# Eddie-Wang1120/Eddie-Wang-Hackathon2023

Measured on AMD Instinct MI355X. Metric: decode tokens/s, whole job (encoder + cross-KV + language-ID + prefill + greedy decode), Whisper large-v2 int8 weight-only + int8 KV; rtf reported beside it, higher is better.
Workload: dtype f16

## Files before the change

### eddie-wang-hackathon2023_amd/csrc/decoder.hip

```cpp
#include <stdio.h>
#include <string.h>

#include <atomic>

#include "engine_internal.h"

using namespace wm;

namespace {
constexpr int MAX_DEVICES = 64;
struct Profiler {
    bool enabled = false; int layer_stride = 1;
    std::vector<hipEvent_t> start, stop; size_t used = 0;
    long long* timeline = nullptr; int timeline_cap = 0;
};
std::mutex g_prof_mu;
Profiler g_prof_dev[MAX_DEVICES];
int current_device_index() {
    int dev = 0;
    if (hipGetDevice(&dev) != hipSuccess || dev < 0 || dev >= MAX_DEVICES) dev = 0;
    return dev;
}

int prof_slot(Profiler& pr, int layer, hipStream_t s) {
// ... 671 lines not shown

int wm_stream_destroy(wm_stream_t stream) {
    if (stream) WM_CHECK_HIP(hipStreamDestroy((hipStream_t)stream));
    return 0;
}

int wm_profile_configure(int enabled, int layer_stride, int max_samples) {
    WM_REQUIRE(layer_stride >= 1 && max_samples >= 0, "wm_profile_configure: bad arguments");
    std::lock_guard<std::mutex> lock(g_prof_mu);
    Profiler& g_prof = g_prof_dev[current_device_index()];
    g_prof.enabled = false;
    for (size_t i = 0; i < g_prof.start.size(); ++i) { (void)hipEventDestroy(g_prof.start[i]); (void)hipEventDestroy(g_prof.stop[i]); }
    g_prof.start.clear(); g_prof.stop.clear(); g_prof.used = 0; g_prof.layer_stride = layer_stride;
    if (!enabled) return 0;
    g_prof.start.resize(max_samples); g_prof.stop.resize(max_samples);
    for (int i = 0; i < max_samples; ++i) {
        WM_CHECK_HIP(hipEventCreate(&g_prof.start[i]));
        WM_CHECK_HIP(hipEventCreate(&g_prof.stop[i]));
    }
    g_prof.enabled = true;
    return 0;
}

int wm_debug_timeline(void* buf, int capacity) {
    std::lock_guard<std::mutex> lock(g_prof_mu);
    Profiler& pr = g_prof_dev[current_device_index()];
    pr.timeline = (long long*)buf;
    pr.timeline_cap = buf ? capacity : 0;
    return 0;
}

int wm_profile_read(double* total_ms, int64_t* count, int reset) {
    WM_REQUIRE(total_ms && count, "wm_profile_read: null argument");
    std::lock_guard<std::mutex> lock(g_prof_mu);
    Profiler& g_prof = g_prof_dev[current_device_index()];
    double sum = 0.0;
    for (size_t i = 0; i < g_prof.used; ++i) {
        float ms = 0.f;
        WM_CHECK_HIP(hipEventSynchronize(g_prof.stop[i]));
        WM_CHECK_HIP(hipEventElapsedTime(&ms, g_prof.start[i], g_prof.stop[i]));
        sum += ms;
    }
    *total_ms = sum; *count = (int64_t)g_prof.used;
    if (reset) g_prof.used = 0;
    return 0;
}

int wm_greedy_step(const wm_greedy_io* io, wm_stream_t stream) {
    WM_REQUIRE(io && io->logits && io->tokens && io->sum_logprobs, "wm_greedy_step: null argument");
    GreedyParams p{};
    p.logits = (h16*)io->logits; p.ld_row = io->row_stride; p.B = io->batch; p.V = io->n_vocab;
    p.tokens = io->tokens; p.ld_tok = io->tokens_ld; p.cur_len = io->cur_len; p.sum_logprobs = io->sum_logprobs;
    p.suppress = io->suppress; p.n_suppress = io->n_suppress; p.blank = io->blank; p.n_blank = io->n_blank;
    p.sample_begin = io->sample_begin; p.eot = io->eot; p.timestamp_begin = io->timestamp_begin;
    p.max_initial_ts = io->max_initial_timestamp_index; p.apply_rules = io->apply_rules; p.n_done = io->n_done;
    p.t_dev = io->n_past_dev;
    p.done = io->done; p.row_limit = io->row_limit;
    WM_REQUIRE(io->temperature >= 0.f, "wm_greedy_step: negative temperature");
    p.temperature = io->temperature; p.seed_lo = (uint32_t)io->seed; p.seed_hi = (uint32_t)(io->seed >> 32);
    p.seed_dev = io->seed_dev; p.row0 = io->row0;
    return launch_greedy(p, (hipStream_t)stream);
}

int wm_step_advance(int32_t* counter, wm_stream_t stream) { return launch_step_advance(counter, (hipStream_t)stream); }
int wm_step_finish(int32_t* counter, const int32_t* done, int batch, int32_t* live, wm_stream_t stream) {
    return launch_step_finish(counter, done, batch, live, (hipStream_t)stream);
}
int wm_step_finish_group(int32_t* counter, const int32_t* done, int batch, int group, int32_t* live, int32_t* live_groups, wm_stream_t stream) {
    return launch_step_finish_group(counter, done, batch, group, live, live_groups, (hipStream_t)stream);
}

int wm_set_rows_path(int min_rows) {
    const int prev = rows_path_min_rows();
    g_rows_min.store(min_rows < 0 ? 0 : min_rows, std::memory_order_relaxed);
    return prev;
}

int wm_set_gemm_small_tiles(int tiles) {
    const int prev = get_gemm_small_tiles();
    set_gemm_small_tiles(tiles);
    return prev;
}

int wm_set_self_attn_waves(int waves) {
    self_attn_waves(1);
    const int prev = g_self_waves.load(std::memory_order_relaxed);
    g_self_waves.store(waves == 1 || waves == 4 ? waves : 0, std::memory_order_relaxed);
    return prev;
}

int wm_set_small_batch_rows(int rows) {
    const int prev = small_path_max_rows();
    g_small_rows.store(rows < 0 ? 0 : (rows > GEMV_SMALL_MAX_M ? GEMV_SMALL_MAX_M : rows), std::memory_order_relaxed);
    return prev;
}

int wm_set_decode_chain(int on) {
    const int prev = g_decode_chain.load(std::memory_order_relaxed);
    g_decode_chain.store(on < 0 ? DECODE_CHAIN_DEFAULT : (on > 2 ? 2 : on), std::memory_order_relaxed);
    for (ChainDev& cd : g_chain_dev) {
        std::lock_guard<std::mutex> lk(cd.mu);
        if (cd.declined) { cd.declined = false; cd.reason.clear(); }
    }
    return prev;
}

int wm_decode_chain_error(int* out) {
    WM_REQUIRE(out, "wm_decode_chain_error: null argument");
    ChainDev& cd = chain_dev_slot(current_device_index());
    const unsigned v = chain_err_peek(cd);
    *out = (int)v;
    if (v) {
        std::lock_guard<std::mutex> lk(cd.mu);
        __atomic_store_n(cd.err_host, 0u, __ATOMIC_RELAXED);
        cd.declined = true;
        cd.reason = "a one-launch decode step gave up waiting for its workgroups (they were not resident together)";
    }
    return 0;
}

int wm_decode_chain_status(wm_chain_status* out) {
    WM_REQUIRE(out, "wm_decode_chain_status: null argument");
    ChainDev& cd = chain_dev_slot(current_device_index());
    std::lock_guard<std::mutex> lk(cd.mu);
    memset(out, 0, sizeof(*out));
    out->mode = g_decode_chain.load(std::memory_order_relaxed);
    out->launches = cd.launches.load(std::memory_order_relaxed);
    out->declined_calls = cd.declined_calls.load(std::memory_order_relaxed);
    out->declined = cd.declined ? 1 : 0;
    out->error_pending = chain_err_peek(cd) ? 1 : 0;
    snprintf(out->reason, sizeof(out->reason), "%s", cd.reason.c_str());
    snprintf(out->footprint, sizeof(out->footprint), "%s", cd.footprint.c_str());
    return 0;
}

int wm_set_cross_v_skip(int on) {
    const int prev = g_cross_v_skip.load(std::memory_order_relaxed);
    g_cross_v_skip.store(on < 0 ? CROSS_V_SKIP_DEFAULT : (on ? 1 : 0), std::memory_order_relaxed);
    return prev;
}

}
```

### eddie-wang-hackathon2023_amd/csrc/gemm_f16.hip

```cpp
#include <stdlib.h>

#include <atomic>

#include "common.h"
#include "kernels.h"

namespace wm {

namespace f16gemm {
constexpr int BK = 64;
}

template <int NWAVE, int BN, int ACT>
__global__ __launch_bounds__(NWAVE * 64, 2) void gemm_f16_kernel(GemmBigParams p) {
    using namespace f16gemm;
    constexpr int TM = 4, ROWS_W = 16 * TM;
    constexpr int BM = NWAVE / 2 * ROWS_W;
    static_assert((BM + BN) / 8 % NWAVE == 0, "DMA pieces must divide evenly over the waves");
    constexpr int A_STAGE = BM * BK * 2, B_STAGE = BN * BK * 2, STAGE = A_STAGE + B_STAGE;
    constexpr int LOADS = (BM + BN) / 8 / NWAVE;
    constexpr int TN = BN / 2 / 16;
    extern __shared__ __attribute__((aligned(1024))) unsigned char smem[];

    const int tid = threadIdx.x, lane = tid & 63, wid = tid >> 6;
// ... 73 lines not shown

    constexpr int WN_COLS = BN / 2;
    const bool scale_cols = p.colscale_n > 0;
    half4v b4[TN];
#pragma unroll
    for (int j = 0; j < TN; ++j) {
        const int col = col0 + wc * WN_COLS + j * 16 + g * 4;
        b4[j] = p.bias ? *(const half4v*)(p.bias + col) : half4v{0, 0, 0, 0};
    }
    const int colw = col0 + wc * WN_COLS + g * 4;
#pragma unroll
    for (int i = 0; i < TM; ++i) {
        const int row = row0 + wr * ROWS_W + i * 16 + (lane & 15);
        const int rowc = row < p.M ? row : p.M - 1;
        half4v r4[TN];
        if (p.residual) {
            const h16* rrow = p.residual + (size_t)(p.res_mod > 0 ? rowc % p.res_mod : rowc) * p.ldr + colw;
#pragma unroll
            for (int j = 0; j < TN; ++j) r4[j] = *(const half4v*)(rrow + j * 16);
        }
        float v[TN][4];
#pragma unroll
        for (int j = 0; j < TN; ++j)
#pragma unroll
            for (int r = 0; r < 4; ++r) v[j][r] = r16_f32(acc[i][j][r] + (float)b4[j][r]);
        if (ACT == 1) {
#pragma unroll
            for (int j = 0; j < TN; ++j)
#pragma unroll
                for (int r = 0; r < 4; ++r) v[j][r] = r16_f32(gelu_erf(v[j][r]));
        } else if (ACT == 2) {
#pragma unroll
            for (int j = 0; j < TN; ++j)
#pragma unroll
                for (int r = 0; r < 4; ++r) v[j][r] = r16_f32(gelu_tanh(v[j][r]));
        }
        if (scale_cols) {
#pragma unroll
            for (int j = 0; j < TN; ++j) {
                const float sc = (colw + j * 16 < p.colscale_n) ? p.colscale : 1.0f;
#pragma unroll
                for (int r = 0; r < 4; ++r) v[j][r] = r16_f32(v[j][r] * sc);
            }
        }
        if (p.residual) {
#pragma unroll
            for (int j = 0; j < TN; ++j)
#pragma unroll
                for (int r = 0; r < 4; ++r) v[j][r] += (float)r4[j][r];
        }
        if (row >= p.M) continue;
        if (p.out_mode == 0) {
            h16* crow = p.C + (p.c_rows > 0 ? (size_t)(row / p.c_rows) * p.c_bstride + (size_t)(row % p.c_rows) * p.ldc
                                            : (size_t)row * p.ldc) + colw;
#pragma unroll
            for (int j = 0; j < TN; ++j)
                *(half4v*)(crow + j * 16) = half4v{(h16)v[j][0], (h16)v[j][1], (h16)v[j][2], (h16)v[j][3]};
        } else {
            const int HC = p.hs_H * 64;
            const int bb = row / p.hs_T, t = row % p.hs_T;
#pragma unroll
            for (int j = 0; j < TN; ++j) {
                const int col = colw + j * 16;
                const int kv = p.hs_kv < 0 ? col / HC : p.hs_kv, cc = p.hs_kv < 0 ? col % HC : col;
                const size_t off = ((((size_t)bb * 2 + kv) * p.hs_H + (cc >> 6)) * p.hs_T + t) * 64 + (cc & 63);
                if (p.q8_inv_scale > 0.f) {
                    char4 q;
                    q.x = (signed char)fminf(127.f, fmaxf(-128.f, rintf(r16(v[j][0]) * p.q8_inv_scale)));
                    q.y = (signed char)fminf(127.f, fmaxf(-128.f, rintf(r16(v[j][1]) * p.q8_inv_scale)));
                    q.z = (signed char)fminf(127.f, fmaxf(-128.f, rintf(r16(v[j][2]) * p.q8_inv_scale)));
                    q.w = (signed char)fminf(127.f, fmaxf(-128.f, rintf(r16(v[j][3]) * p.q8_inv_scale)));
                    *(char4*)((signed char*)p.C + off) = q;
                } else
                *(half4v*)(p.C + off) = half4v{(h16)v[j][0], (h16)v[j][1], (h16)v[j][2], (h16)v[j][3]};
            }
        }
    }
}

static std::atomic<int> g_small_tiles{GEMM_SMALL_TILES_DEFAULT};
void set_gemm_small_tiles(int tiles) { g_small_tiles.store(tiles > 0 ? tiles : (tiles == 0 ? 0 : GEMM_SMALL_TILES_DEFAULT), std::memory_order_relaxed); }
int get_gemm_small_tiles() { return g_small_tiles.load(std::memory_order_relaxed); }

int launch_gemm_f16(const GemmBigParams& p, hipStream_t stream) {
    using namespace f16gemm;
    const bool few = p.max_wgs <= 0 && p.N % 128 == 0 &&
                     (long)((p.M + 255) / 256) * ((p.N + 255) / 256) < (long)g_small_tiles.load(std::memory_order_relaxed);
    if (!few && gemm_f16p_supports(p)) return launch_gemm_f16p(p, stream);
    WM_REQUIRE(p.N % 128 == 0, "gemm_f16: N=%d must be a multiple of 128", p.N);
    WM_REQUIRE(p.K % BK == 0, "gemm_f16: K=%d must be a multiple of %d", p.K, BK);
    WM_REQUIRE(p.lda % 8 == 0, "gemm_f16: lda=%d must be a multiple of 8 (16-byte loads)", p.lda);
    WM_REQUIRE(p.ldc % 4 == 0 && p.ldr % 4 == 0, "gemm_f16: ldc/ldr must be multiples of 4 (8-byte epilogue accesses)");
    WM_REQUIRE(p.M > 0, "gemm_f16: empty M");
    WM_REQUIRE(p.act >= 0 && p.act <= 2, "gemm_f16: act=%d", p.act);
    static const int tiny_max = lab_env_int("WM_GEMM_TINY_TILES", GEMM_TINY_TILES_DEFAULT);
    const long tiles128 = (long)((p.M + 127) / 128) * (p.N / 128);
    const int form = few ? (tiles128 <= tiny_max ? 3 : 2) : (p.N % 256 == 0 ? 0 : 1);
    const int bm = form == 3 ? 64 : (form == 2 ? 128 : 256), bn = form == 0 ? 256 : 128;
    const int grid = ((p.M + bm - 1) / bm) * (p.N / bn);
    static std::atomic<unsigned long long> attr_set{0};
    int dev = 0;
    WM_CHECK_HIP(hipGetDevice(&dev));
    const int slot = dev & 63;
    using Kern = void (*)(GemmBigParams);
    static const Kern kerns[4][3] = {{gemm_f16_kernel<8, 256, 0>, gemm_f16_kernel<8, 256, 1>, gemm_f16_kernel<8, 256, 2>},
                                     {gemm_f16_kernel<8, 128, 0>, gemm_f16_kernel<8, 128, 1>, gemm_f16_kernel<8, 128, 2>},
                                     {gemm_f16_kernel<4, 128, 0>, gemm_f16_kernel<4, 128, 1>, gemm_f16_kernel<4, 128, 2>},
                                     {gemm_f16_kernel<2, 128, 0>, gemm_f16_kernel<2, 128, 1>, gemm_f16_kernel<2, 128, 2>}};
    static const int rows_of[4] = {256, 256, 128, 64}, cols_of[4] = {256, 128, 128, 128};
    const unsigned long long bit = 1ull << slot;
    if (!(attr_set.load(std::memory_order_acquire) & bit)) {
        for (int f = 0; f < 4; ++f)
            for (int a = 0; a < 3; ++a)
                WM_CHECK_HIP(hipFuncSetAttribute((const void*)kerns[f][a], hipFuncAttributeMaxDynamicSharedMemorySize,
                                                 2 * (rows_of[f] + cols_of[f]) * BK * 2));
        attr_set.fetch_or(bit, std::memory_order_release);
    }
    const size_t lds = (size_t)2 * (bm + bn) * BK * 2;
    hipLaunchKernelGGL(kerns[form][p.act], dim3(grid), dim3(form == 3 ? 128 : (form == 2 ? 256 : 512)), lds, stream, p);
    WM_LAUNCH_CHECK(stream, "gemm_f16");
    return 0;
}

__global__ void dequant_w8_kernel(const int8_t* q, const h16* scale, h16* out, int N, int K) {
    const size_t total = (size_t)N * K / 8;
    for (size_t i = blockIdx.x * (size_t)blockDim.x + threadIdx.x; i < total; i += (size_t)gridDim.x * blockDim.x) {
        const size_t e = i * 8;
        const h16 s = scale[e / K];
        const uint2 w = *(const uint2*)(q + e);
        half2v h[4];
        cvt_s8x4_f16x4(w.x, h[0], h[1]);
        cvt_s8x4_f16x4(w.y, h[2], h[3]);
        half8v o;
#pragma unroll
        for (int j = 0; j < 4; ++j) { o[2 * j] = h[j][0] * s; o[2 * j + 1] = h[j][1] * s; }
        *(half8v*)(out + e) = o;
    }
}

int launch_dequant_w8(const int8_t* q, const h16* scale, h16* out, int N, int K, hipStream_t stream) {
    WM_REQUIRE(K % 8 == 0, "dequant_w8: K=%d must be a multiple of 8", K);
    hipLaunchKernelGGL(dequant_w8_kernel, dim3(2048), dim3(256), 0, stream, q, scale, out, N, K);
    WM_LAUNCH_CHECK(stream, "dequant_w8");
    return 0;
}

}
```

### eddie-wang-hackathon2023_amd/csrc/kernels.h

```cpp
#pragma once
#include "common.h"

namespace wm {

struct GemmBigParams {
    const h16* A; int lda; int M; int K;
    const void* W; int N;
    const h16* bias;
    h16* C; int ldc;
    const h16* residual; int ldr; int res_mod;
    int act;
    int colscale_n; float colscale;
    int out_mode;
    int hs_T, hs_H, hs_kv;
    float q8_inv_scale;
    int a_rows; long a_bstride;
    int c_rows; long c_bstride;
    int max_wgs;
    int nt_flags;
    int tile_rows;
};
int launch_gemm_f16(const GemmBigParams& p, hipStream_t stream);
constexpr int GEMM_SMALL_TILES_DEFAULT = 150;
constexpr int GEMM_TINY_TILES_DEFAULT = 160;
void set_gemm_small_tiles(int tiles);
int get_gemm_small_tiles();
int launch_gemm_f16p(const GemmBigParams& p, hipStream_t stream);
bool gemm_f16p_supports(const GemmBigParams& p);
int launch_dequant_w8(const int8_t* q, const h16* scale, h16* out, int N, int K, hipStream_t stream);

struct GemmSkinnyParams {
    const h16* A; int lda; int M; int K;
    const void* Wt; int n_blocks; int w8;
    const h16* scale;
    int ksplit;
    float* part;
    long part_sstride;
    h16* out; int ldc; int n_valid;
};
constexpr int SKINNY_MAX_M = 256;
int launch_gemm_skinny(const GemmSkinnyParams& p, hipStream_t stream);
int skinny_default_ksplit(int M, int K, int n_blocks, int w8);

struct GemvSmallParams {
    const h16* A; int lda; int M; int K;
    const void* Wt; int n_blocks; int w8;
    const h16* scale;
    int ksplit;
    const h16* ln_g; const h16* ln_b;
    int mode;
    const h16* bias; int gelu_kind;
    float* out32; int ld32;
    h16* out16; int ld16; int n_valid;
    h16* x; int ldx;
};
constexpr int GEMV_SMALL_MAX_M = 32;
int launch_gemv_small(const GemvSmallParams& p, hipStream_t stream);

constexpr int CHAIN_MAX_STAGES = 6;
constexpr int CHAIN_MAX_ROWS = 8;
constexpr int DECODE_CHAIN_DEFAULT = 2;
struct ChainStage {
    const void* Wt; const h16* scale; const h16* bias;
    const h16* ln_g; const h16* ln_b;
    int K, n_blocks;
    int mode;
    int pad_;
};
struct ChainLayerStatic { const h16* qkv_bias; const h16* cq_bias; float kv_scale; int pad_; };
struct ChainLayerIo { const void* cross_kv; void* cache; };
struct GemvChainParams {
    int n_stages; const ChainStage* st;
    float* out32;
    int w8, gelu_kind;
    h16* x;
    unsigned long long* gran_x; unsigned long long* gran_h;
    const h16* cross_kv; int cross_Tk, cross_heads, cross_nsplit; const h16* cross_qbias;
    unsigned long long* gran_q;
    int cross_at, merge_at, merge_nsplit, merge_heads;
    unsigned long long* gran_p;
    const float* self_part; const h16* self_bias; void* self_cache; int self_cap, self_T, self_heads, self_i8; const int32_t* self_t_dev;
    float self_kv_scale; h16* self_out; unsigned long long* gran_c;
    int n_layers; const ChainLayerStatic* lstat; const ChainLayerIo* lio; unsigned long long* gran_s;
    int rows; long cross_row_bytes, self_row_bytes;
    const int32_t* live;
    unsigned* err;
    const unsigned* generation; int launch_id;
};
bool gemv_chain_supports(int C, int w8, int n_cu);
int gemv_chain_resident(int w8, int self_i8, int rows, int cross_Tk, int cross_nsplit, int n_wg, int n_cu, bool* ok, char* why, size_t why_cap);
int launch_occupy(int n_wg, size_t lds_bytes, long long usec, hipStream_t stream);
int launch_gemv_chain(const GemvChainParams& p, const ChainStage* host_stages, int n_wg, hipStream_t stream);
int launch_chain_io_table(ChainLayerIo* dst, const ChainLayerIo* host, int n, hipStream_t stream);

bool gemm_rows_supports(int K, int w8);
int launch_gemm_rows(const GemvSmallParams& p, hipStream_t stream);

struct RowFinishParams {
    const float* part; int ksplit; int M; int N; int ldp;
    long part_sstride;
    const h16* bias;
    int mode; int gelu_kind;
    h16* x; int ldx;
    const h16* ln_g; const h16* ln_b;
    h16* out; int ldo;
    int eager;
};
int launch_row_finish(const RowFinishParams& p, hipStream_t stream);

struct EmbedParams {
    const int32_t* tokens; int tokens_ld;
// ... 127 lines not shown
```

### eddie-wang-hackathon2023_amd/native.py

```python
from __future__ import annotations

import atexit
import ctypes as C
import os
from typing import Optional, Sequence

import sys
import warnings


def _hip_already_initialised() -> bool:
    t = sys.modules.get("torch")
    try:
        return bool(t is not None and t.cuda.is_initialized())
    except Exception:
        return False


def _configure_runtime() -> dict:
    name = "DEBUG_CLR_GRAPH_PACKET_CAPTURE"
    late = _hip_already_initialised()
    if name in os.environ:
        return {"name": name, "value": os.environ[name], "set_by": "caller", "in_time": None}
    if os.environ.get("WM_GRAPH_NODE_REPLAY", "1") == "0":
        return {"name": name, "value": None, "set_by": "nobody (WM_GRAPH_NODE_REPLAY=0)", "in_time": None}
    os.environ[name] = "0"
    if late:
        warnings.warn("whisper_mi355: the HIP runtime was initialised before this package was imported, so "
                      f"{name}=0 (node-by-node graph replay, 6-10 % of the small-batch token step) is NOT in effect: "
                      "import the package before the first torch.cuda call, or export the variable yourself", RuntimeWarning, stacklevel=3)
    return {"name": name, "value": "0", "set_by": "package", "in_time": not late}


RUNTIME_KNOBS = _configure_runtime()


def runtime_report() -> dict:
    rep = dict(RUNTIME_KNOBS)
    rep["effective_env"] = os.environ.get(RUNTIME_KNOBS["name"])
    if _lib is not None:
        buf = C.create_string_buffer(4096)
        _lib.wm_lab_knobs(buf, 4096)
        rep["lab_knobs_honoured"] = buf.value.decode() or None
    return rep


_HERE = os.path.dirname(os.path.abspath(__file__))
LIB_PATH = os.environ.get("WM_LIBRARY_PATH") or os.path.join(_HERE, "libwhisper_mi355.so")

EXPORTS = (
    "wm_version", "wm_last_error", "wm_device_count", "wm_engine_create", "wm_engine_destroy",
    "wm_engine_info", "wm_engine_weight_bytes", "wm_encoder_workspace_bytes", "wm_encoder_forward",
    "wm_encoder_forward_shared", "wm_encoder_forward_range",
    "wm_cross_kv_workspace_bytes", "wm_cross_kv", "wm_decoder_workspace_bytes", "wm_decoder_step",
    "wm_greedy_step", "wm_gemm", "wm_gemm_skinny", "wm_gemm_skinny_default_ksplit", "wm_layernorm",
    "wm_attn_encoder", "wm_attn_decode_cross", "wm_attn_decode_self", "wm_quantize_i8",
    "wm_profile_configure", "wm_profile_read", "wm_step_advance", "wm_log_mel_workspace_bytes", "wm_log_mel",
    "wm_flac_info", "wm_flac_decode", "wm_conv1d_gelu", "wm_argmax", "wm_gemv_fused", "wm_gemm_rows", "wm_set_rows_path", "wm_set_small_batch_rows", "wm_set_self_attn_waves", "wm_set_gemm_small_tiles", "wm_lab_knobs", "wm_set_cross_v_skip", "wm_set_decode_chain", "wm_decode_chain_error", "wm_decode_chain_status", "wm_debug_occupy", "wm_decoder_step_multi", "wm_stream_create_cu_mask", "wm_stream_destroy", "wm_attn_decode_cross_i8", "wm_debug_timeline",
    "wm_step_finish",
    "wm_beam_workspace_bytes", "wm_beam_step", "wm_kv_reorder",
    "wm_gemm_ex", "wm_row_finish", "wm_embed", "wm_mel_transpose_pad", "wm_zero_pad_rows",
    "wm_decoder_step_tap", "wm_align_workspace_bytes", "wm_align", "wm_dtw_workspace_bytes", "wm_dtw",
    "wm_mel_windows", "wm_resample", "wm_attn_decode_self_rows",
    "wm_attn_self_ex", "wm_attn_cross_ex",
    "wm_forced_probs",
    "wm_section_cuts_workspace_bytes", "wm_section_cuts",
    "wm_step_finish_group", "wm_attn_cross_group_ex", "wm_decoder_step_group",
    "wm_decoder_prefill_workspace_bytes", "wm_decoder_prefill", "wm_attn_prefill_self", "wm_attn_prefill_cross",
)


ABI_VERSION = 8

import threading as _threading
CAPTURE_LOCK = _threading.RLock()


class WmError(RuntimeError):
    pass


class WmFlacStreamInfo(C.Structure):
    _fields_ = [("sample_rate", C.c_int32), ("channels", C.c_int32), ("bits_per_sample", C.c_int32),
                ("max_block_size", C.c_int32), ("total_samples", C.c_int64), ("md5", C.c_uint8 * 16)]


class WmChainStatus(C.Structure):
    _fields_ = [("mode", C.c_int32), ("declined", C.c_int32), ("error_pending", C.c_int32), ("pad_", C.c_int32),
                ("launches", C.c_int64), ("declined_calls", C.c_int64), ("reason", C.c_char * 200), ("footprint", C.c_char * 200)]


def chain_status() -> dict:
    st = WmChainStatus()
    check(load_library().wm_decode_chain_status(C.byref(st)), "wm_decode_chain_status")
    return {"mode": st.mode, "declined": bool(st.declined), "error_pending": bool(st.error_pending), "launches": int(st.launches),
            "declined_calls": int(st.declined_calls), "reason": st.reason.decode(), "footprint": st.footprint.decode()}


class WmDims(C.Structure):
    _fields_ = [(n, C.c_int32) for n in (
        "n_mels", "n_audio_ctx", "n_audio_state", "n_audio_head", "n_audio_layer",
        "n_vocab", "n_text_ctx", "n_text_state", "n_text_head", "n_text_layer")]

    def to_dict(self):
        return {n: int(getattr(self, n)) for n, _ in self._fields_}


class WmDecoderIO(C.Structure):
    _fields_ = [
        ("batch", C.c_int32), ("n_new", C.c_int32), ("n_past", C.c_int32),
        ("tokens", C.c_void_p), ("tokens_ld", C.c_int32), ("positional_embedding", C.c_void_p),
        ("past", C.POINTER(C.c_void_p)), ("past_capacity", C.c_int32),
        ("present", C.POINTER(C.c_void_p)), ("present_capacity", C.c_int32),
        ("cross", C.POINTER(C.c_void_p)),
        ("logits", C.c_void_p),
        ("workspace", C.c_void_p), ("workspace_bytes", C.c_size_t),
        ("qkv_amax", C.c_void_p),
        ("n_past_dev", C.c_void_p),
        ("live_rows", C.c_void_p),
        ("workspace_id", C.c_uint64),
        ("not_alone", C.c_int32),
        ("row_start", C.c_void_p),
    ]


class WmDecoderGroupIO(C.Structure):
    _fields_ = [("io", WmDecoderIO), ("cross_group", C.c_int32), ("live_groups", C.c_void_p)]


class WmPrefillIO(C.Structure):
    _fields_ = [("io", WmDecoderIO), ("logits_from", C.c_int32)]


class WmGemvIO(C.Structure):
    _fields_ = [
        ("a", C.c_void_p), ("lda", C.c_int32), ("m", C.c_int32), ("k", C.c_int32),
        ("wt", C.c_void_p), ("n_blocks", C.c_int32), ("w8", C.c_int32), ("scale", C.c_void_p),
        ("ln_gamma", C.c_void_p), ("ln_beta", C.c_void_p),
        ("mode", C.c_int32), ("bias", C.c_void_p), ("gelu_kind", C.c_int32),
        ("out32", C.c_void_p), ("ld32", C.c_int32),
        ("out16", C.c_void_p), ("ld16", C.c_int32), ("n_valid", C.c_int32),
# ... 105 lines not shown
    ]


class WmAttnCrossGroupIO(C.Structure):
    _fields_ = WmAttnCrossIO._fields_ + [("G", C.c_int32), ("live_utt", C.c_void_p)]


class WmTapIO(C.Structure):
    _fields_ = [("q_tape", C.c_void_p), ("capacity", C.c_int32), ("heads", C.POINTER(C.c_int32)), ("n_heads", C.c_int32)]


class WmAlignIO(C.Structure):
    _fields_ = [
        ("engine", C.c_void_p),
        ("batch", C.c_int32), ("n_text_head", C.c_int32), ("n_audio_ctx", C.c_int32),
        ("q_tape", C.c_void_p), ("capacity", C.c_int32),
        ("cross", C.POINTER(C.c_void_p)), ("n_layers", C.c_int32),
        ("heads", C.POINTER(C.c_int32)), ("n_heads", C.c_int32),
        ("n_tokens", C.c_void_p),
        ("n_frames", C.c_void_p),
        ("n_prefix", C.c_int32), ("filter_width", C.c_int32),
        ("cap_tokens", C.c_int32),
        ("matrix", C.c_void_p), ("ld", C.c_int32),
        ("path_text", C.c_void_p), ("path_time", C.c_void_p),
        ("path_len", C.c_void_p),
        ("workspace", C.c_void_p), ("workspace_bytes", C.c_size_t),
    ]


_lib: Optional[C.CDLL] = None


def load_library(path: str = LIB_PATH) -> C.CDLL:
    global _lib
    if _lib is not None:
        return _lib
    if not os.path.exists(path):
        raise WmError(f"{path} not found: build it with `python __graft_entry__.py` "
                      f"(hipcc --offload-arch=gfx950); there is no fallback path")
    lib = C.CDLL(path, mode=C.RTLD_GLOBAL)
    for name in EXPORTS:
        if not hasattr(lib, name):
            raise WmError(f"{path} does not export {name}")
    vp, i32, sz = C.c_void_p, C.c_int, C.c_size_t
    lib.wm_version.restype = i32
    if lib.wm_version() != ABI_VERSION:
        raise WmError(f"{path} has ABI version {lib.wm_version()}, this binding needs {ABI_VERSION}: rebuild it "
                      f"(python __graft_entry__.py)")
    lib.wm_last_error.restype = C.c_char_p
    lib.wm_device_count.argtypes = [C.POINTER(i32)]
    lib.wm_engine_create.argtypes = [vp, sz, i32, C.POINTER(vp)]
    lib.wm_engine_destroy.argtypes = [vp]
    lib.wm_engine_destroy.restype = None
    lib.wm_engine_info.argtypes = [vp, C.POINTER(C.c_int32), C.POINTER(C.c_uint32), C.POINTER(WmDims)]
    lib.wm_engine_weight_bytes.argtypes = [vp]
    lib.wm_engine_weight_bytes.restype = sz
    lib.wm_encoder_workspace_bytes.argtypes = [vp, i32]
    lib.wm_encoder_workspace_bytes.restype = sz
    lib.wm_encoder_forward.argtypes = [vp, vp, i32, vp, vp, sz, vp]
    lib.wm_encoder_forward_shared.argtypes = [vp, vp, i32, vp, vp, sz, i32, vp]
    lib.wm_encoder_forward_range.argtypes = [vp, vp, i32, vp, vp, sz, i32, i32, i32, vp]
    lib.wm_cross_kv_workspace_bytes.argtypes = [vp, i32]
    lib.wm_cross_kv_workspace_bytes.restype = sz
    lib.wm_cross_kv.argtypes = [vp, vp, i32, C.POINTER(vp), vp, sz, vp]
    lib.wm_decoder_workspace_bytes.argtypes = [vp, i32, i32]
    lib.wm_decoder_workspace_bytes.restype = sz
    lib.wm_decoder_step.argtypes = [vp, C.POINTER(WmDecoderIO), vp]
    lib.wm_decoder_step_group.argtypes = [vp, C.POINTER(WmDecoderGroupIO), vp]
    lib.wm_decoder_prefill_workspace_bytes.restype = C.c_size_t
    lib.wm_decoder_prefill_workspace_bytes.argtypes = [vp, i32, i32]
    lib.wm_decoder_prefill.argtypes = [vp, C.POINTER(WmPrefillIO), vp]
    lib.wm_attn_prefill_self.argtypes = [vp, i32, i32, i32, vp, i32, i32, C.c_float, vp, vp, vp, vp]
    lib.wm_attn_prefill_cross.argtypes = [vp, i32, i32, i32, i32, vp, vp, vp, vp]
    lib.wm_greedy_step.argtypes = [C.POINTER(WmGreedyIO), vp]
    lib.wm_gemm.argtypes = [vp, i32, i32, i32, vp, i32, i32, vp, vp, vp, i32, i32, vp, i32, vp, sz, vp]
    lib.wm_conv1d_gelu.argtypes = [vp, i32, i32, i32, vp, i32, vp, i32, i32, i32, vp, vp]
    lib.wm_argmax.argtypes = [vp, C.c_int64, i32, i32, vp, vp]
    lib.wm_gemv_fused.argtypes = [C.POINTER(WmGemvIO), vp]
    lib.wm_set_small_batch_rows.argtypes = [i32]
    lib.wm_gemm_rows.argtypes = [C.POINTER(WmGemvIO), vp]
    lib.wm_set_rows_path.argtypes = [i32]
    lib.wm_set_self_attn_waves.argtypes = [i32]
    lib.wm_set_gemm_small_tiles.argtypes = [i32]
    lib.wm_lab_knobs.argtypes = [C.c_char_p, sz]
    lib.wm_set_cross_v_skip.argtypes = [i32]
    lib.wm_set_decode_chain.argtypes = [i32]
    lib.wm_decode_chain_error.argtypes = [C.POINTER(C.c_int)]
    lib.wm_decode_chain_status.argtypes = [C.POINTER(WmChainStatus)]
    lib.wm_debug_occupy.argtypes = [i32, sz, C.c_int64, vp]
    lib.wm_gemm_skinny.argtypes = [vp, i32, i32, i32, vp, i32, i32, vp, i32, vp, vp]
    lib.wm_gemm_skinny_default_ksplit.argtypes = [i32, i32, i32, i32]
    lib.wm_layernorm.argtypes = [vp, i32, i32, i32, vp, vp, vp, i32, vp]
    lib.wm_attn_encoder.argtypes = [vp, i32, i32, i32, i32, vp, i32, vp]
    lib.wm_attn_decode_cross.argtypes = [vp, i32, i32, i32, i32, vp, vp, i32, vp, vp]
    lib.wm_attn_decode_self.argtypes = [vp, i32, i32, i32, i32, vp, i32, vp, i32, i32, C.c_float, vp, vp]
    lib.wm_attn_decode_self_rows.argtypes = [vp, i32, i32, i32, i32, vp, i32, i32, C.c_float, vp, vp, vp, vp]
    lib.wm_quantize_i8.argtypes = [vp, vp, C.c_int64, C.c_float, vp]
    lib.wm_log_mel_workspace_bytes.argtypes = [i32, i32, i32]
    lib.wm_log_mel_workspace_bytes.restype = sz
    lib.wm_log_mel.argtypes = [vp, i32, i32, C.c_int64, vp, i32, vp, vp, vp, sz, vp]
    lib.wm_decoder_step_multi.argtypes = [vp, i32, C.POINTER(C.POINTER(WmDecoderIO)), C.POINTER(vp), vp]
    lib.wm_stream_create_cu_mask.argtypes = [C.POINTER(C.c_uint32), i32, C.POINTER(vp)]
    lib.wm_stream_destroy.argtypes = [vp]
    lib.wm_attn_decode_cross_i8.argtypes = [vp, i32, i32, i32, i32, vp, C.c_float, vp, i32, vp, vp]
    lib.wm_flac_info.argtypes = [vp, sz, C.POINTER(WmFlacStreamInfo)]
    lib.wm_flac_decode.argtypes = [vp, sz, vp, C.c_int64, C.POINTER(C.c_int64)]
    lib.wm_step_advance.argtypes = [vp, vp]
    lib.wm_step_finish.argtypes = [vp, vp, i32, vp, vp]
    lib.wm_beam_workspace_bytes.argtypes = [i32, i32]
    lib.wm_beam_workspace_bytes.restype = sz
    lib.wm_beam_step.argtypes = [C.POINTER(WmBeamIO), vp]
    lib.wm_kv_reorder.argtypes = [vp, i32, i32, i32, i32, i32, i32, vp, vp, i32, vp, vp]
    lib.wm_debug_timeline.argtypes = [vp, i32]
    lib.wm_gemm_ex.argtypes = [C.POINTER(WmGemmIO), vp]
    lib.wm_row_finish.argtypes = [C.POINTER(WmRowFinishIO), vp]
    lib.wm_attn_self_ex.argtypes = [C.POINTER(WmAttnSelfIO), vp]
    lib.wm_attn_cross_ex.argtypes = [C.POINTER(WmAttnCrossIO), vp]
    lib.wm_attn_cross_group_ex.argtypes = [C.POINTER(WmAttnCrossGroupIO), vp]
    lib.wm_step_finish_group.argtypes = [vp, vp, i32, i32, vp, vp, vp]
    lib.wm_embed.argtypes = [vp, i32, i32, i32, vp, i32, vp, vp, i32, i32, vp, vp, vp]
    lib.wm_mel_transpose_pad.argtypes = [vp, i32, i32, i32, vp, vp]
    lib.wm_zero_pad_rows.argtypes = [vp, i32, i32, i32, vp]
    lib.wm_mel_windows.argtypes = [vp, vp, vp, i32, i32, i32, vp, vp]
    lib.wm_resample.argtypes = [vp, i32, i32, C.c_int64, C.c_float, vp, i32, i32, i32, vp, C.c_int64, vp]
    lib.wm_forced_probs.argtypes = [vp, i32, i32, i32, C.c_int64, C.c_int64, i32, vp, i32, vp, i32, vp]
    lib.wm_section_cuts_workspace_bytes.argtypes = [i32, C.c_int64]
    lib.wm_section_cuts_workspace_bytes.restype = sz
    lib.wm_section_cuts.argtypes = [vp, vp, vp, i32, i32, i32, i32, i32, vp, i32, vp, vp, sz, C.c_int64, vp]
    lib.wm_decoder_step_tap.argtypes = [vp, C.POINTER(WmDecoderIO), C.POINTER(WmTapIO), vp]
    lib.wm_align_workspace_bytes.argtypes = [i32, i32, i32, i32]
    lib.wm_align_workspace_bytes.restype = sz
    lib.wm_align.argtypes = [C.POINTER(WmAlignIO), vp]
    lib.wm_dtw_workspace_bytes.argtypes = [i32, i32, i32]
    lib.wm_dtw_workspace_bytes.restype = sz
    lib.wm_dtw.argtypes = [vp, i32, C.c_int64, i32, vp, vp, i32, i32, vp, vp, i32, vp, vp, sz, vp]
    lib.wm_profile_configure.argtypes = [i32, i32, i32]
    lib.wm_profile_read.argtypes = [C.POINTER(C.c_double), C.POINTER(C.c_int64), i32]
    _lib = lib
    return lib


def check(rc: int, what: str = ""):
    if rc != 0:
        msg = load_library().wm_last_error().decode(errors="replace")
        raise WmError(f"{what or 'libwhisper_mi355'} failed (rc={rc}): {msg}")


def ptr_array(tensors: Sequence) -> "C.Array":
    arr = (C.c_void_p * len(tensors))()
    for i, t in enumerate(tensors):
        arr[i] = None if t is None else (t.data_ptr() if hasattr(t, "data_ptr") else int(t))
    return arr


class Engine:

    def __init__(self, blob: bytes, device: int = 0):
        self.lib = load_library()
        handle = C.c_void_p()
        if not isinstance(blob, bytes):
            blob = bytes(blob)
        check(self.lib.wm_engine_create(C.cast(C.c_char_p(blob), C.c_void_p), len(blob), device, C.byref(handle)),
              "wm_engine_create")
        self.handle = handle
        kind, flags, dims = C.c_int32(), C.c_uint32(), WmDims()
        check(self.lib.wm_engine_info(self.handle, C.byref(kind), C.byref(flags), C.byref(dims)))
# ... 51 lines not shown
```

### include/whisper_mi355.h

```cpp
#ifndef WHISPER_MI355_H
#define WHISPER_MI355_H

#include <stddef.h>
#include <stdint.h>

#ifdef __cplusplus
extern "C" {
#endif

typedef struct wm_engine wm_engine;
typedef void* wm_stream_t;

enum { WM_ENGINE_ENCODER = 0, WM_ENGINE_DECODER = 1, WM_ENGINE_CROSS_KV = 2 };
enum { WM_FLAG_WEIGHT_ONLY_INT8 = 1, WM_FLAG_INT8_KV = 2, WM_FLAG_GELU_TANH = 4,
       WM_FLAG_INT8_CROSS_KV = 16  };

typedef struct wm_dims {
    int32_t n_mels, n_audio_ctx, n_audio_state, n_audio_head, n_audio_layer;
    int32_t n_vocab, n_text_ctx, n_text_state, n_text_head, n_text_layer;
} wm_dims;

#define WM_ABI_VERSION 8
int wm_version(void);
const char* wm_last_error(void);
// ... 155 lines not shown
typedef struct wm_row_finish_io {
    const float* part; int32_t ksplit, m, n, ldp; int64_t part_sstride;
    const void* bias;
    int32_t mode, gelu_kind;
    void* x; int32_t ldx;
    const void* ln_gamma; const void* ln_beta;
    void* out; int32_t ldo;
} wm_row_finish_io;
int wm_row_finish(const wm_row_finish_io* io, wm_stream_t stream);
typedef struct wm_attn_self_io {
    const float* part; int32_t ksplit, ldp; int64_t part_sstride;
    const void* bias;
    int32_t B, L, T, H;
    const void* past; int64_t past_bstride; int32_t past_cap;
    void* present; int64_t present_bstride; int32_t present_cap;
    int32_t int8_kv; float kv_scale;
    float* amax;
    const int32_t* t_dev;
    void* out; int32_t ldo;
    const int32_t* live;
    const int32_t* row_start;
    int32_t waves;
} wm_attn_self_io;
int wm_attn_self_ex(const wm_attn_self_io* io, wm_stream_t stream);
typedef struct wm_attn_cross_io {
    const float* part; int32_t ksplit, ldp; int64_t part_sstride;
    const void* bias;
    int32_t B, L, H, Tk;
    const void* kv; int64_t kv_bstride;
    float kv_q8_scale;
    void* out; int32_t ldo;
    int32_t nsplit;
    float* ws;
    const int32_t* live;
    int32_t skip_zero_rows;
} wm_attn_cross_io;
int wm_attn_cross_ex(const wm_attn_cross_io* io, wm_stream_t stream);
typedef struct wm_attn_cross_group_io {
    const float* part; int32_t ksplit, ldp; int64_t part_sstride;
    const void* bias;
    int32_t B, L, H, Tk;
    const void* kv; int64_t kv_bstride;
    float kv_q8_scale;
    void* out; int32_t ldo;
    int32_t nsplit;
    float* ws;
    const int32_t* live;
    int32_t skip_zero_rows;
    int32_t G;
    const int32_t* live_utt;
} wm_attn_cross_group_io;
int wm_attn_cross_group_ex(const wm_attn_cross_group_io* io, wm_stream_t stream);
int wm_embed(const int32_t* tokens, int tokens_ld, int M, int L, const void* emb_tiles, int C, const void* pos,
             void* x, int ldx, int n_vocab, const int32_t* t_dev, uint32_t* generation, wm_stream_t stream);
int wm_mel_transpose_pad(const void* mel, int B, int n_mels, int T, void* out, wm_stream_t stream);
int wm_mel_windows(const void* const* src, const int32_t* src_frames, const int32_t* seek, int batch, int n_mels, int n_window,
                   void* out, wm_stream_t stream);
int wm_forced_probs(const void* logits, int batch, int n_pos, int n_vocab, int64_t stride_b, int64_t stride_p, int limit,
                    const int32_t* next, int next_ld, float* out, int out_ld, wm_stream_t stream);
size_t wm_section_cuts_workspace_bytes(int batch, int64_t total_frames);
int wm_section_cuts(const void* const* src, const int32_t* src_ld, const int32_t* content, int batch, int n_mels, int lo, int hi,
                    int h, int32_t* cuts, int cuts_ld, int32_t* n_cuts, void* workspace, size_t workspace_bytes,
                    int64_t total_frames, wm_stream_t stream);
int wm_zero_pad_rows(void* buf, int B, int Tpad, int C, wm_stream_t stream);
int wm_argmax(const void* logits, int64_t row_stride, int batch, int n_vocab, int32_t* ids, wm_stream_t stream);
int wm_gemm_skinny(const void* A, int lda, int M, int K, const void* Wt, int n_blocks, int w8,
                   const void* scale, int ksplit, float* part, wm_stream_t stream);
int wm_gemm_skinny_default_ksplit(int M, int K, int n_blocks, int w8);
typedef struct wm_gemv_io {
    const void* a; int32_t lda, m, k;
    const void* wt; int32_t n_blocks, w8; const void* scale;
    const void* ln_gamma; const void* ln_beta;
    int32_t mode; const void* bias; int32_t gelu_kind;
    float* out32; int32_t ld32;
    void* out16; int32_t ld16, n_valid;
    void* x; int32_t ldx;
} wm_gemv_io;
int wm_gemv_fused(const wm_gemv_io* io, wm_stream_t stream);
int wm_set_small_batch_rows(int rows);
int wm_gemm_rows(const wm_gemv_io* io, wm_stream_t stream);
int wm_set_rows_path(int min_rows);
int wm_set_self_attn_waves(int waves);
int wm_set_gemm_small_tiles(int tiles);
typedef struct wm_chain_status {
    int32_t mode;
    int32_t declined;
    int32_t error_pending;
    int32_t pad_;
    int64_t launches;
    int64_t declined_calls;
    char reason[200];
    char footprint[200];
} wm_chain_status;
int wm_set_decode_chain(int on);
int wm_decode_chain_error(int* out);
int wm_decode_chain_status(wm_chain_status* out);
int wm_debug_occupy(int n_workgroups, size_t lds_bytes, int64_t microseconds, wm_stream_t stream);
int wm_set_cross_v_skip(int on);
int wm_lab_knobs(char* buf, size_t cap);
int wm_layernorm(const void* x, int ldx, int M, int N, const void* gamma, const void* beta,
                 void* out, int ldo, wm_stream_t stream);
int wm_attn_encoder(const void* qkv, int ld, int B, int T, int H, void* out, int ldo, wm_stream_t stream);
int wm_attn_decode_cross(const float* q, int B, int L, int H, int Tk, const void* kv, void* out,
                         int nsplit, float* ws, wm_stream_t stream);
int wm_attn_decode_cross_i8(const float* q, int B, int L, int H, int Tk, const void* kv_i8, float kv_scale,
                            void* out, int nsplit, float* ws, wm_stream_t stream);
int wm_attn_decode_self(const float* qkv, int B, int L, int T, int H, const void* past, int past_cap,
                        void* present, int present_cap, int int8_kv, float kv_scale, void* out,
                        wm_stream_t stream);
int wm_attn_prefill_self(const float* qkv, int B, int L, int H, void* cache, int cap, int int8_kv, float kv_scale, void* out,
                         const int32_t* row_start, const int32_t* live_rows, wm_stream_t stream);
int wm_attn_prefill_cross(const float* q, int B, int L, int H, int Tk, const void* kv, void* out, const int32_t* live_rows,
                          wm_stream_t stream);
int wm_attn_decode_self_rows(const float* qkv, int B, int L, int T, int H, void* cache, int cap, int int8_kv, float kv_scale,
                             void* out, const int32_t* row_start, const int32_t* live_rows, wm_stream_t stream);
int wm_quantize_i8(const void* x, void* q, int64_t n, float inv_scale, wm_stream_t stream);

size_t wm_log_mel_workspace_bytes(int batch, int n_samples, int n_mels);
int wm_log_mel(const float* audio, int batch, int n_samples, int64_t audio_ld, const float* filters,
               int n_mels, void* mel_f16, float* mel_f32, void* workspace, size_t workspace_bytes,
               wm_stream_t stream);

int wm_resample(const void* pcm, int dtype, int channels, int64_t n_in, float scale, const float* table, int L, int M, int half,
                float* out, int64_t n_out, wm_stream_t stream);

typedef struct wm_flac_streaminfo {
    int32_t sample_rate;
    int32_t channels;
    int32_t bits_per_sample;
    int32_t max_block_size;
    int64_t total_samples;
    uint8_t md5[16];
} wm_flac_streaminfo;
int wm_flac_info(const void* data, size_t bytes, wm_flac_streaminfo* info);
int wm_flac_decode(const void* data, size_t bytes, int32_t* pcm, int64_t capacity_samples,
                   int64_t* n_decoded);

int wm_profile_configure(int enabled, int layer_stride, int max_samples);
int wm_profile_read(double* total_ms, int64_t* count, int reset);
int wm_debug_timeline(void* buf, int capacity);

#ifdef __cplusplus
}
#endif
#endif
```

Before: 16760.

## Add persistent 256x256 f16 GEMM kernel for encoder residual projections

Adds a new persistent 4-wave GEMM kernel with 256x256 tiles. It double-buffers global-to-LDS loads interleaved with MFMA issue, maps tiles XCD-aware with row grouping, and keeps bias in LDS. By default it is routed only for encoder-sized shapes (N=1280, K=1280 or 5120) that use a residual epilogue, i.e. the attention output and MLP down projections. The aim is better data reuse and overlap than the existing f16p/f16 kernels. The cost is a large new hand-scheduled kernel with high LDS use and one wave per SIMD, which could lower latency hiding.

```diff
diff --git a/eddie-wang-hackathon2023_amd/csrc/decoder.hip b/eddie-wang-hackathon2023_amd/csrc/decoder.hip
--- a/eddie-wang-hackathon2023_amd/csrc/decoder.hip
+++ b/eddie-wang-hackathon2023_amd/csrc/decoder.hip
@@ -777,6 +777,9 @@
     return prev;
 }
 
+int wm_set_gemm_wave_form(int mode) { return set_gemm_wave_form(mode); }
+int64_t wm_gemm_wave_form_launches(void) { return (int64_t)gemm_wave_form_launches(); }
+
 int wm_set_self_attn_waves(int waves) {
     self_attn_waves(1);
     const int prev = g_self_waves.load(std::memory_order_relaxed);
diff --git a/eddie-wang-hackathon2023_amd/csrc/gemm_f16.hip b/eddie-wang-hackathon2023_amd/csrc/gemm_f16.hip
--- a/eddie-wang-hackathon2023_amd/csrc/gemm_f16.hip
+++ b/eddie-wang-hackathon2023_amd/csrc/gemm_f16.hip
@@ -179,10 +179,33 @@
 void set_gemm_small_tiles(int tiles) { g_small_tiles.store(tiles > 0 ? tiles : (tiles == 0 ? 0 : GEMM_SMALL_TILES_DEFAULT), std::memory_order_relaxed); }
 int get_gemm_small_tiles() { return g_small_tiles.load(std::memory_order_relaxed); }
 
+struct WaveFormShape { int N, K, epilogue; };
+static constexpr WaveFormShape WAVE_FORM_SHAPES[] = {
+    {1280, 1280, 2},
+    {1280, 5120, 2},
+};
+static std::atomic<int> g_wave_form{0};
+static std::atomic<long> g_wave_form_launches{0};
+long gemm_wave_form_launches() { return g_wave_form_launches.load(std::memory_order_relaxed); }
+int set_gemm_wave_form(int mode) { return g_wave_form.exchange(mode == 1 || mode == 2 ? mode : 0, std::memory_order_relaxed); }
+static bool takes_wave_form(const GemmBigParams& p) {
+    const int mode = g_wave_form.load(std::memory_order_relaxed);
+    if (mode == 1 || !gemm_f16w_supports(p)) return false;
+    if (mode == 2) return true;
+    const int epilogue = p.act == 1 ? 1 : (p.residual ? 2 : 0);
+    for (const WaveFormShape& s : WAVE_FORM_SHAPES)
+        if (s.N == p.N && s.K == p.K && s.epilogue == epilogue) return true;
+    return false;
+}
+
 int launch_gemm_f16(const GemmBigParams& p, hipStream_t stream) {
     using namespace f16gemm;
     const bool few = p.max_wgs <= 0 && p.N % 128 == 0 &&
                      (long)((p.M + 255) / 256) * ((p.N + 255) / 256) < (long)g_small_tiles.load(std::memory_order_relaxed);
+    if (!few && takes_wave_form(p)) {
+        g_wave_form_launches.fetch_add(1, std::memory_order_relaxed);
+        return launch_gemm_f16w(p, stream);
+    }
     if (!few && gemm_f16p_supports(p)) return launch_gemm_f16p(p, stream);
     WM_REQUIRE(p.N % 128 == 0, "gemm_f16: N=%d must be a multiple of 128", p.N);
     WM_REQUIRE(p.K % BK == 0, "gemm_f16: K=%d must be a multiple of %d", p.K, BK);
diff --git a/eddie-wang-hackathon2023_amd/csrc/gemm_f16w.hip b/eddie-wang-hackathon2023_amd/csrc/gemm_f16w.hip
--- /dev/null
+++ b/eddie-wang-hackathon2023_amd/csrc/gemm_f16w.hip
@@ -0,0 +1,272 @@
+#include <stdlib.h>
+
+#include <atomic>
+#include <type_traits>
+
+#include "common.h"
+#include "kernels.h"
+
+namespace wm {
+
+namespace f16w {
+constexpr int BM = 256, BN = 256, BK = 64, NWAVE = 4;
+constexpr int A_PART = BM * BK * 2, SLOT = (BM + BN) * BK * 2;
+constexpr int MAX_N = 8192;
+}
+
+template <int ACT>
+__global__ __launch_bounds__(256) void gemm_f16w_kernel(GemmBigParams p) {
+    using namespace f16w;
+    extern __shared__ __attribute__((aligned(1024))) unsigned char smem[];
+    const int tid = threadIdx.x, lane = tid & 63, wid = __builtin_amdgcn_readfirstlane(tid >> 6);
+    const int wr = wid >> 1, wc = wid & 1;
+    const int g = lane >> 4;
+
+    const int nt_n = p.N / BN, nt_m = (p.M + BM - 1) / BM, n_tiles = nt_n * nt_m;
+    const int per_xcd = gridDim.x >> 3;
+    const int xcd = blockIdx.x & 7, j0 = blockIdx.x >> 3;
+    const int band = (n_tiles + 7) >> 3;
+    const int lo = min(n_tiles, xcd * band), hi = min(n_tiles, lo + band);
+    const int my_tiles = (hi - lo - j0 + per_xcd - 1) > 0 ? (hi - lo - j0 + per_xcd - 1) / per_xcd : 0;
+    if (my_tiles == 0) return;
+    const int nk = p.K / BK;
+    const int R = p.tile_rows > 0 ? p.tile_rows : max(1, min(8, (int)((2816u << 10) / ((unsigned)p.K * BM * 2u))));
+    const int row_first = (lo + nt_n - 1) / nt_n, row_last = hi / nt_n;
+    const int q_head = min(hi, row_first * nt_n) - lo, q_mid = max(0, row_last - row_first) * nt_n;
+    auto tile_of = [&](int q, int& tm, int& tn) {
+        if (q < q_head) { const int tile = lo + q; tm = tile / nt_n; tn = tile - tm * nt_n; return; }
+        const int q2 = q - q_head;
+        if (q2 >= q_mid) { const int tile = row_last * nt_n + (q2 - q_mid); tm = tile / nt_n; tn = tile - tm * nt_n; return; }
+        const int sr = q2 / (R * nt_n), rem = q2 - sr * (R * nt_n);
+        const int rows_here = min(R, (row_last - row_first) - sr * R);
+        tn = rem / rows_here;
+        tm = row_first + sr * R + (rem - tn * rows_here);
+    };
+
+    const unsigned char* a_base = nullptr;
+    const unsigned char* w_base = nullptr;
+    uint32_t a_lane[8], w_lane0;
+    {
+        const int r = wid * 8 + (lane >> 3);
+        const int c = (lane & 7) ^ ((r >> 1) & 7);
+        w_lane0 = (uint32_t)r * (uint32_t)p.K * 2u + c * 16;
+    }
+    auto set_tile = [&](int t) {
+        int tm, tn;
+        tile_of(j0 + t * per_xcd, tm, tn);
+        a_base = (const unsigned char*)(p.A + (size_t)tm * BM * p.lda);
+        w_base = (const unsigned char*)p.W + (size_t)tn * BN * p.K * 2;
+        int ll;
+        asm volatile("v_mbcnt_lo_u32_b32 %0, -1, 0\n\tv_mbcnt_hi_u32_b32 %0, -1, %0" : "=v"(ll));
+        const int r0 = wid * 8 + (ll >> 3);
+        const int c = (ll & 7) ^ ((r0 >> 1) & 7);
+        const int last = p.M - 1 - tm * BM;
+#pragma unroll
+        for (int q = 0; q < 8; ++q) a_lane[q] = (uint32_t)min(r0 + 32 * q, last) * (uint32_t)p.lda * 2u + c * 16;
+    };
+    int load_ks = 0, load_tile = 0;
+    auto issue_piece = [&](uint32_t slot, int q) {
+        if (q < 8) {
+            __builtin_amdgcn_global_load_lds((const __attribute__((address_space(1))) void*)(a_base + a_lane[q]),
+                                             (__attribute__((address_space(3))) void*)(smem + slot + (wid + NWAVE * q) * 1024), 16, 0, 0);
+        } else {
+            uint32_t w_lane = w_lane0 + (uint32_t)(q - 8) * 64u * (uint32_t)p.K;
+            asm volatile("" : "+v"(w_lane));
+            __builtin_amdgcn_global_load_lds((const __attribute__((address_space(1))) void*)(w_base + w_lane),
+                                             (__attribute__((address_space(3))) void*)(smem + slot + A_PART + (wid + NWAVE * (q - 8)) * 1024), 16, 0, 0);
+        }
+    };
+    auto advance_loader = [&]() {
+        a_base += BK * 2; w_base += BK * 2;
+        if (++load_ks == nk) { load_ks = 0; ++load_tile; set_tile(load_tile < my_tiles ? load_tile : my_tiles - 1); }
+    };
+    set_tile(0);
+#pragma unroll
+    for (int q = 0; q < 16; ++q) issue_piece(0, q);
+    advance_loader();
+
+    {
+        h16* bias_lds0 = (h16*)(smem + 2 * SLOT);
+        for (int c = tid; c < p.N; c += 256) bias_lds0[c] = p.bias ? p.bias[c] : (h16)0.f;
+    }
+
+    const int sw = ((lane & 15) >> 1) & 7;
+    const int a_off0 = (wr * 128 + (lane & 15)) * 128, b_off0 = A_PART + (wc * 128 + (lane & 15)) * 128;
+    const int ch0 = (g ^ sw) << 4;
+
+    float4v acc[8][8];
+    half8v af[2][8], bx[2][8];
+    auto read_frag = [&](auto set_tag, const unsigned char* st, int ch, int n) {
+        constexpr int S = decltype(set_tag)::value;
+        if (n == 0) bx[S][0] = *(const half8v*)(st + b_off0 + ch);
+        else if (n == 1) af[S][0] = *(const half8v*)(st + a_off0 + ch);
+        else if (n < 9) bx[S][n - 1] = *(const half8v*)(st + b_off0 + ch + (n - 1) * 2048);
+        else af[S][n - 8] = *(const half8v*)(st + a_off0 + ch + (n - 8) * 2048);
+    };
+
+    asm volatile("s_waitcnt vmcnt(0) lgkmcnt(0)" ::: "memory");
+    __builtin_amdgcn_s_barrier();
+    __builtin_amdgcn_sched_barrier(0);
+#pragma unroll
+    for (int q = 0; q < 16; ++q) issue_piece(SLOT, q);
+    advance_loader();
+#pragma unroll
+    for (int n = 0; n < 16; ++n) read_frag(std::integral_constant<int, 0>{}, smem, ch0, n);
+
+    uint32_t cons_slot = 0;
+    int t = 0;
+    auto step = [&](auto half_tag, auto first_tag) {
+        constexpr int HALF = decltype(half_tag)::value;
+        constexpr bool FIRST = decltype(first_tag)::value;
+        const unsigned char* nxt = smem + (HALF ? (cons_slot ^ SLOT) : cons_slot);
+        const int nch = HALF ? ch0 : (ch0 ^ 64);
+#pragma unroll
+        for (int m = 0; m < 64; ++m) {
+            const int i = m >> 3, j = m & 7;
+            acc[i][j] = __builtin_amdgcn_mfma_f32_16x16x32_f16(bx[HALF][j], af[HALF][i], FIRST ? float4v{0.f, 0.f, 0.f, 0.f} : acc[i][j], 0, 0, 0);
+            __builtin_amdgcn_sched_barrier(0);
+            if (HALF == 0 && m < 32 && (m & 1) == 0) read_frag(std::integral_constant<int, 1 - HALF>{}, nxt, nch, m >> 1);
+            if (HALF == 1 && (m & 3) == 3) read_frag(std::integral_constant<int, 1 - HALF>{}, nxt, nch, m >> 2);
+            if (HALF == 1 && (m & 3) == 1) issue_piece(cons_slot, m >> 2);
+            __builtin_amdgcn_sched_barrier(0);
+        }
+    };
+    auto slot = [&](auto first_tag) {
+        step(std::integral_constant<int, 0>{}, first_tag);
+        asm volatile("s_waitcnt vmcnt(0) lgkmcnt(0)" ::: "memory");
+        __builtin_amdgcn_s_barrier();
+        __builtin_amdgcn_sched_barrier(0);
+        step(std::integral_constant<int, 1>{}, std::false_type{});
+        advance_loader();
+        cons_slot ^= SLOT;
+    };
+    for (;;) {
+        slot(std::true_type{});
+#pragma unroll 1
+        for (int ks = 1; ks < nk; ++ks) slot(std::false_type{});
+
+        int tm, tn;
+        tile_of(j0 + t * per_xcd, tm, tn);
+        const int row0 = tm * BM, col0 = tn * BN;
+        int le;
+        asm volatile("v_mbcnt_lo_u32_b32 %0, -1, 0\n\tv_mbcnt_hi_u32_b32 %0, -1, %0" : "=v"(le));
+        const int ge = le >> 4, rl = le & 15;
+        const int colw = col0 + wc * 128 + ge * 4;
+        const h16* bias_lds = (const h16*)(smem + 2 * SLOT) + colw;
+        auto finish = [&](auto res_tag) {
+            constexpr bool RES = decltype(res_tag)::value;
+            const int odd = ge & 1;
+            const int colx = col0 + wc * 128 + 4 * (ge - odd) + 16 * odd;
+            float2v bf[8][2];
+#pragma unroll
+            for (int j = 0; j < 8; ++j) {
+                const half4v b4 = *(const half4v*)(bias_lds + j * 16);
+                bf[j][0] = float2v{(float)b4[0], (float)b4[1]};
+                bf[j][1] = float2v{(float)b4[2], (float)b4[3]};
+            }
+            auto block = [&](int i, int j, uint32_t& lo, uint32_t& hi) {
+                float2v v0 = float2v{acc[i][j][0], acc[i][j][1]} + bf[j][0];
+                float2v v1 = float2v{acc[i][j][2], acc[i][j][3]} + bf[j][1];
+                half2v h0 = __builtin_convertvector(v0, half2v), h1 = __builtin_convertvector(v1, half2v);
+                if constexpr (ACT == 1) {
+                    v0 = __builtin_convertvector(h0, float2v); v1 = __builtin_convertvector(h1, float2v);
+                    v0 = gelu_erf2(v0); v1 = gelu_erf2(v1);
+                    h0 = __builtin_convertvector(v0, half2v); h1 = __builtin_convertvector(v1, half2v);
+                }
+                lo = __builtin_bit_cast(uint32_t, h0); hi = __builtin_bit_cast(uint32_t, h1);
+            };
+#pragma unroll
+            for (int hb = 0; hb < 2; ++hb) {
+                uint4 r8[RES ? 4 : 1][RES ? 4 : 1];
+                if constexpr (RES) {
+#pragma unroll
+                    for (int ii = 0; ii < 4; ++ii) {
+                        const int row = row0 + wr * 128 + (hb * 4 + ii) * 16 + rl;
+                        const h16* rrow = p.residual + (size_t)(row < p.M ? row : p.M - 1) * p.ldr + colx;
+#pragma unroll
+                        for (int jp = 0; jp < 4; ++jp) r8[ii][jp] = *(const uint4*)(rrow + jp * 32);
+                    }
+                    __builtin_amdgcn_sched_barrier(0);
+                }
+#pragma unroll
+                for (int ii = 0; ii < 4; ++ii) {
+                    const int i = hb * 4 + ii;
+                    const int row = row0 + wr * 128 + i * 16 + rl;
+                    h16* crow = p.C + (size_t)(row < p.M ? row : p.M - 1) * p.ldc + colx;
+#pragma unroll
+                    for (int jp = 0; jp < 4; ++jp) {
+                        uint32_t a0, a1, b0, b1;
+                        block(i, 2 * jp, a0, a1);
+                        block(i, 2 * jp + 1, b0, b1);
+                        lane_rows_swap16(a0, b0);
+                        lane_rows_swap16(a1, b1);
+                        uint4 o = make_uint4(a0, a1, b0, b1);
+                        if constexpr (RES) {
+                            const half8v x = __builtin_bit_cast(half8v, o), r = __builtin_bit_cast(half8v, r8[ii][jp]);
+                            half8v y;
+#pragma unroll
+                            for (int e = 0; e < 8; e += 2) {
+                                const float2v s2 = float2v{(float)x[e], (float)x[e + 1]} + float2v{(float)r[e], (float)r[e + 1]};
+                                const half2v h = __builtin_convertvector(s2, half2v);
+                                y[e] = h[0]; y[e + 1] = h[1];
+                            }
+                            o = __builtin_bit_cast(uint4, y);
+                        }
+                        if (row < p.M) *(uint4*)(crow + jp * 32) = o;
+                    }
+                    __builtin_amdgcn_sched_barrier(0);
+                }
+            }
+        };
+        if constexpr (ACT != 0) {
+            finish(std::false_type{});
+        } else {
+            if (p.residual) finish(std::true_type{}); else finish(std::false_type{});
+        }
+        if (++t == my_tiles) break;
+    }
+    asm volatile("s_waitcnt vmcnt(0)" ::: "memory");
+}
+
+bool gemm_f16w_supports(const GemmBigParams& p) {
+    using namespace f16w;
+    return p.N % BN == 0 && p.N <= MAX_N && p.K % BK == 0 && p.K >= 128 && p.M > 0 && p.max_wgs <= 0 &&
+           (p.act == 0 || (p.act == 1 && !p.residual)) && p.colscale_n <= 0 && p.out_mode == 0 && p.q8_inv_scale <= 0.f &&
+           p.a_rows == 0 && p.c_rows == 0 && p.res_mod == 0 &&
+           p.lda % 8 == 0 && ((uintptr_t)p.A & 15) == 0 && ((uintptr_t)p.W & 15) == 0 &&
+           p.ldc % 8 == 0 && ((uintptr_t)p.C & 15) == 0 && (!p.residual || (p.ldr % 8 == 0 && ((uintptr_t)p.residual & 15) == 0));
+}
+
+int launch_gemm_f16w(const GemmBigParams& p, hipStream_t stream) {
+    using namespace f16w;
+    WM_REQUIRE(gemm_f16w_supports(p), "gemm_f16w: unsupported call (N=%d K=%d act=%d)", p.N, p.K, p.act);
+    static std::atomic<int> n_cu_dev[64];
+    int dev = 0;
+    WM_CHECK_HIP(hipGetDevice(&dev));
+    const int slot = (dev >= 0 && dev < 64) ? dev : 0;
+    int n_cu = n_cu_dev[slot].load(std::memory_order_relaxed);
+    using Kern = void (*)(GemmBigParams);
+    static const Kern kerns[2] = {gemm_f16w_kernel<0>, gemm_f16w_kernel<1>};
+    constexpr size_t LDS_BYTES = (size_t)2 * SLOT + MAX_N * 2;
+    if (n_cu == 0) {
+        int v = 0;
+        WM_CHECK_HIP(hipDeviceGetAttribute(&v, hipDeviceAttributeMultiprocessorCount, dev));
+        n_cu = v > 0 ? v : 256;
+        for (int a = 0; a < 2; ++a)
+            WM_CHECK_HIP(hipFuncSetAttribute((const void*)kerns[a], hipFuncAttributeMaxDynamicSharedMemorySize, (int)LDS_BYTES));
+        n_cu_dev[slot].store(n_cu, std::memory_order_relaxed);
+    }
+    const int n_tiles = ((p.M + BM - 1) / BM) * (p.N / BN);
+    int grid = (n_cu / 8) * 8;
+    if (grid < 8) grid = 8;
+    const int need = ((n_tiles + 7) / 8) * 8;
+    if (grid > need) grid = need;
+    static const int lab_rows = lab_env_int("WM_GEMM_TILE_ROWS", 0);
+    GemmBigParams q = p;
+    if (q.tile_rows <= 0) q.tile_rows = lab_rows;
+    hipLaunchKernelGGL(kerns[p.act], dim3(grid), dim3(256), LDS_BYTES, stream, q);
+    WM_LAUNCH_CHECK(stream, "gemm_f16w");
+    return 0;
+}
+
+}
diff --git a/eddie-wang-hackathon2023_amd/csrc/kernels.h b/eddie-wang-hackathon2023_amd/csrc/kernels.h
--- a/eddie-wang-hackathon2023_amd/csrc/kernels.h
+++ b/eddie-wang-hackathon2023_amd/csrc/kernels.h
@@ -27,6 +27,10 @@
 int get_gemm_small_tiles();
 int launch_gemm_f16p(const GemmBigParams& p, hipStream_t stream);
 bool gemm_f16p_supports(const GemmBigParams& p);
+int launch_gemm_f16w(const GemmBigParams& p, hipStream_t stream);
+bool gemm_f16w_supports(const GemmBigParams& p);
+long gemm_wave_form_launches();
+int set_gemm_wave_form(int mode);
 int launch_dequant_w8(const int8_t* q, const h16* scale, h16* out, int N, int K, hipStream_t stream);
 
 struct GemmSkinnyParams {
diff --git a/eddie-wang-hackathon2023_amd/native.py b/eddie-wang-hackathon2023_amd/native.py
--- a/eddie-wang-hackathon2023_amd/native.py
+++ b/eddie-wang-hackathon2023_amd/native.py
@@ -56,7 +56,7 @@
     "wm_greedy_step", "wm_gemm", "wm_gemm_skinny", "wm_gemm_skinny_default_ksplit", "wm_layernorm",
     "wm_attn_encoder", "wm_attn_decode_cross", "wm_attn_decode_self", "wm_quantize_i8",
     "wm_profile_configure", "wm_profile_read", "wm_step_advance", "wm_log_mel_workspace_bytes", "wm_log_mel",
-    "wm_flac_info", "wm_flac_decode", "wm_conv1d_gelu", "wm_argmax", "wm_gemv_fused", "wm_gemm_rows", "wm_set_rows_path", "wm_set_small_batch_rows", "wm_set_self_attn_waves", "wm_set_gemm_small_tiles", "wm_lab_knobs", "wm_set_cross_v_skip", "wm_set_decode_chain", "wm_decode_chain_error", "wm_decode_chain_status", "wm_debug_occupy", "wm_decoder_step_multi", "wm_stream_create_cu_mask", "wm_stream_destroy", "wm_attn_decode_cross_i8", "wm_debug_timeline",
+    "wm_flac_info", "wm_flac_decode", "wm_conv1d_gelu", "wm_argmax", "wm_gemv_fused", "wm_gemm_rows", "wm_set_rows_path", "wm_set_small_batch_rows", "wm_set_self_attn_waves", "wm_set_gemm_small_tiles", "wm_set_gemm_wave_form", "wm_gemm_wave_form_launches", "wm_lab_knobs", "wm_set_cross_v_skip", "wm_set_decode_chain", "wm_decode_chain_error", "wm_decode_chain_status", "wm_debug_occupy", "wm_decoder_step_multi", "wm_stream_create_cu_mask", "wm_stream_destroy", "wm_attn_decode_cross_i8", "wm_debug_timeline",
     "wm_step_finish",
     "wm_beam_workspace_bytes", "wm_beam_step", "wm_kv_reorder",
     "wm_gemm_ex", "wm_row_finish", "wm_embed", "wm_mel_transpose_pad", "wm_zero_pad_rows",
@@ -328,6 +328,9 @@
     lib.wm_set_rows_path.argtypes = [i32]
     lib.wm_set_self_attn_waves.argtypes = [i32]
     lib.wm_set_gemm_small_tiles.argtypes = [i32]
+    lib.wm_set_gemm_wave_form.argtypes = [i32]
+    lib.wm_gemm_wave_form_launches.argtypes = []
+    lib.wm_gemm_wave_form_launches.restype = C.c_int64
     lib.wm_lab_knobs.argtypes = [C.c_char_p, sz]
     lib.wm_set_cross_v_skip.argtypes = [i32]
     lib.wm_set_decode_chain.argtypes = [i32]
diff --git a/include/whisper_mi355.h b/include/whisper_mi355.h
--- a/include/whisper_mi355.h
+++ b/include/whisper_mi355.h
@@ -261,6 +261,8 @@
 int wm_set_rows_path(int min_rows);
 int wm_set_self_attn_waves(int waves);
 int wm_set_gemm_small_tiles(int tiles);
+int wm_set_gemm_wave_form(int mode);
+int64_t wm_gemm_wave_form_launches(void);
 typedef struct wm_chain_status {
     int32_t mode;
     int32_t declined;
```

Result: no change. 16750 (-0.0%).
